# prashanthr05/bipedal-locomotion-framework

Hardware: AMD Instinct MI355X
Metric: DCM-MPC QP solves/sec (batch, horizon=100) at 1/2/4/8 MI355X (higher is better)
Workload: dtype f64; 1 GPU; configs[1]: batch=4096 DCM-MPC QPs per GPU, horizon=100, M=8 facet slots, fp64, one wavefront per QP; batch_per_gpu=4096, global_batch=4096, horizon=100, max_facets=8, parallelism=shard1 (independent problems)

## Files before the change

### bipedal-locomotion-framework_amd/csrc/dcm_mpc_as.hip

```cpp
#include "dcm_qp_common.h"
#include "dcm_mpc_ipm_body.h"

#include <stdlib.h>

#include <type_traits>

namespace blf {
namespace {
using namespace qp;

#ifdef BLF_STAMPS
__device__ unsigned long long g_as_stamps[32];
__device__ unsigned long long g_as_timeline[65536 * 4];
__device__ unsigned long long g_as32_timeline[65536 * 4];
#define AS_STAMP(t) unsigned long long t = __builtin_amdgcn_s_memtime()
#define AS_STAMP_ADD(slot, t0) \
    do { if (blockIdx.x < 64 && threadIdx.x == 0) atomicAdd(&g_as_stamps[slot], __builtin_amdgcn_s_memtime() - (t0)); } while (0)
#define AS_COUNT(slot) \
    do { if (blockIdx.x < 64 && threadIdx.x == 0) atomicAdd(&g_as_stamps[slot], 1ull); } while (0)
#else
#define AS_STAMP(t)
#define AS_STAMP_ADD(slot, t0)
#define AS_COUNT(slot)
#endif
// ... 64 lines not shown

constexpr int kAsMinWaves = 2;

template <class T>
struct Row {
    T x, y, b;
};

template <class T, class RS>
__device__ __forceinline__ Row<T> row(const RS& R, int i, int col)
{
    const int o = R.at(i, col);
    const auto a = R.A2[o];
    return {T(a.x), T(a.y), T(R.Bv[o])};
}

template <class T, class RS>
__device__ __forceinline__ Row<T> normal(const RS& R, int i, int col)
{
    const auto a = R.A2[R.at(i, col)];
    return {T(a.x), T(a.y), T(0)};
}

struct NoRows {};
template <int KPL>
struct RegRows {
    Row<float> v[KPL][kMaxFacets];
};
template <class RR>
constexpr bool kHasRows = !std::is_same<RR, NoRows>::value;

template <int KPL, class RS>
__device__ __forceinline__ void load_rows(RegRows<KPL>& rr, const RS& R, int N, int M, int lane)
{
#pragma unroll
    for (int j = 0; j < KPL; ++j) {
        const int col = KPL * lane + j < N ? R.col(j, lane) : 0;
#pragma unroll
        for (int i = 0; i < kMaxFacets; ++i) rr.v[j][i] = row<float>(R, i < M ? i : 0, col);
    }
}
template <int KPL, class RS>
__device__ __forceinline__ void load_rows(NoRows&, const RS&, int, int, int)
{
}



enum : int { kTreeKS = 0, kTreePad = 1, kTreeDpp = 2 };

template <int KPL, int TR>
__device__ __forceinline__ void assume_pad(int N)
{
    if (KPL == 2 && TR != kTreeDpp) __builtin_assume((TR == kTreePad) == (N <= 2 * kWave - 2));
}

template <class T, int KPL>
constexpr bool kPairFloat = sizeof(T) == 4 && KPL == 2;

template <int L, bool FWD, class T>
__device__ __forceinline__ void aff_level(T& g0, T& g1, T& g2, T& g3, T& e0, T& e1, int lane)
{
    T p0, p1, p2, p3, q0, q1;
    if constexpr (FWD) {
        p0 = tree_fwd<L>(g0); p1 = tree_fwd<L>(g1); p2 = tree_fwd<L>(g2);
        p3 = tree_fwd<L>(g3); q0 = tree_fwd<L>(e0); q1 = tree_fwd<L>(e1);
// ... 155 lines not shown
    K.qx0 = q0 * (K.x0 - K.xr0);
    K.qx1 = q1 * (K.x1 - K.xr1);
}

template <bool SEL, class T>
__device__ __forceinline__ void rc_knot(RcT<T>& e, bool own, T al, const T (&E)[3], const PT<T>& P)
{
    if constexpr (SEL) {
        const T a = own ? al : T(1);
        e.a0 = a; e.a1 = T(0); e.a2 = T(0); e.a3 = a;
        e.g0 = E[0]; e.g1 = E[1]; e.g2 = E[2];
        e.h0 = own ? P.Qw0 : T(0); e.h1 = T(0); e.h2 = own ? P.Qw1 : T(0);
    } else if (own) {
        e.a0 = al; e.a1 = T(0); e.a2 = T(0); e.a3 = al;
        e.g0 = E[0]; e.g1 = E[1]; e.g2 = E[2];
        e.h0 = P.Qw0; e.h1 = T(0); e.h2 = P.Qw1;
    } else {
        e.a0 = T(1); e.a1 = T(0); e.a2 = T(0); e.a3 = T(1);
        e.g0 = e.g1 = e.g2 = T(0);
        e.h0 = e.h1 = e.h2 = T(0);
    }
}

template <int KPL, int TR, class T>
__device__ __forceinline__ bool as_riccati(AKnotT<T> (&K)[KPL], const PT<T>& P, const T (&E)[KPL][3], int N,
                                           int lane)
{
    bool ok = true;
    RcT<T> e;
    rc_knot<kPairFloat<T, KPL>>(e, KPL * lane < N, K[0].al, E[0], P);
    if constexpr (KPL == 2) {
        RcT<T> e1;
        rc_knot<kPairFloat<T, KPL>>(e1, KPL * lane + 1 < N, K[1].al, E[1], P);
        ok = rc_combine(e, e1) && ok;
    }
    const int ln = opaque(lane);
    constexpr bool pad = KPL == 2 && TR == kTreePad;
    auto level = [&](int ad, RcT<T>& q) {
        q.a0 = bperm(ad, e.a0); q.a1 = bperm(ad, e.a1); q.a2 = bperm(ad, e.a2); q.a3 = bperm(ad, e.a3);
        q.g0 = bperm(ad, e.g0); q.g1 = bperm(ad, e.g1); q.g2 = bperm(ad, e.g2);
        q.h0 = bperm(ad, e.h0); q.h1 = bperm(ad, e.h1); q.h2 = bperm(ad, e.h2);
    };
    auto level1 = [&](RcT<T>& q) {
        constexpr int C = pad ? kNextKeep : kNextWrap;
        q.a0 = dpp1<C>(e.a0); q.a1 = dpp1<C>(e.a1); q.a2 = dpp1<C>(e.a2); q.a3 = dpp1<C>(e.a3);
        q.g0 = dpp1<C>(e.g0); q.g1 = dpp1<C>(e.g1); q.g2 = dpp1<C>(e.g2);
        q.h0 = dpp1<C>(e.h0); q.h1 = dpp1<C>(e.h1); q.h2 = dpp1<C>(e.h2);
    };
    if constexpr (TR == kTreeDpp) {
        rc_tree<0>(e, ok, lane);
        rc_tree<1>(e, ok, lane);
        rc_tree<2>(e, ok, lane);
        rc_tree<3>(e, ok, lane);
        rc_tree<4>(e, ok, lane);
        rc_tree<5>(e, ok, lane);
    } else {
        {
// ... 4 lines not shown
#pragma unroll
        for (int d = 2; d < kWave; d <<= 1) {
            RcT<T> q;
            level(ks_addr<pad, false>(ln, d), q);
            if (ks_has<pad, false>(ln, d)) ok = rc_combine(e, q) && ok;
        }
    }
    T P00, P01, P11;
    ok = rc_apply(e, P.Pw0, T(0), P.Pw1, P00, P01, P11) && ok;
    T Pn00 = dpp1<kNextWrap>(P00), Pn01 = dpp1<kNextWrap>(P01), Pn11 = dpp1<kNextWrap>(P11);
    if (lane == kWave - 1) {
        Pn00 = P.Pw0;
        Pn01 = T(0);
        Pn11 = P.Pw1;
    }
    constexpr int L = KPL - 1;
    K[L].P00 = Pn00;
    K[L].P01 = Pn01;
    K[L].P11 = Pn11;
    if constexpr (KPL == 2) {
        RcT<T> e1;
        rc_knot<kPairFloat<T, KPL>>(e1, KPL * lane + 1 < N, K[1].al, E[1], P);
        T o00, o01, o11;
        ok = rc_apply(e1, Pn00, Pn01, Pn11, o00, o01, o11) && ok;
        K[0].P00 = o00;
        K[0].P01 = o01;
        K[0].P11 = o11;
    }
#pragma unroll
    for (int j = 0; j < KPL; ++j) {
        if (KPL * lane + j == N - 1) {
            K[j].P00 = P.Pw0;
            K[j].P01 = T(0);
            K[j].P11 = P.Pw1;
        }
    }
    return ok;
}

template <int KPL, int TR, class T>
__device__ __forceinline__ void as_solve(const AKnotT<T> (&K)[KPL], const T (&g)[KPL][2], int N, int lane,
                                         T (&dr)[KPL][2], T (&dx)[KPL][2], T (&vn)[KPL][2])
{
    constexpr bool kSel = kPairFloat<T, KPL>;
    T G[KPL][4], c[KPL][2], y[KPL][2];
#pragma unroll
    for (int j = 0; j < KPL; ++j) {
        const bool own = KPL * lane + j < N;
        if constexpr (!kSel) {
            G[j][0] = G[j][1] = G[j][2] = G[j][3] = T(0);
            c[j][0] = c[j][1] = y[j][0] = y[j][1] = T(0);
        }
        if (kSel || own) {
            const AKnotT<T>& Kj = K[j];
            const T b2 = Kj.be * Kj.be;
            const T ab = Kj.al * Kj.be;
            const T m00 = FD2(Kj.P00, Kj.h00, Kj.P01, Kj.h01);
            const T m01 = FD2(Kj.P00, Kj.h01, Kj.P01, Kj.h11);
            const T m10 = FD2(Kj.P01, Kj.h00, Kj.P11, Kj.h01);
            const T m11 = FD2(Kj.P01, Kj.h01, Kj.P11, Kj.h11);
// ... 538 lines not shown

template <class T, class RS>
__device__ __forceinline__ void as_pass_h(AKnotT<T>& K, const PT<T>& P, const RS& R, int col, int pk,
                                          bool& okp, const Row<T>& na)
{
    const int pc = pk & 3, pi1 = (pk >> 2) & 15;
    const T b2 = K.be * K.be;
    const T B00 = fma(b2, K.P00, P.Rw0);
    const T B01 = b2 * K.P01;
    const T B11 = fma(b2, K.P11, P.Rw1);
    Row<T> a = na;
    if constexpr (!kCarryNormals<T>) a = normal<T>(R, pi1, opaque(col));
    const T u = a.y * a.y, v = a.x * a.x, q = a.x * a.y;
    const T detB = fma(B00, B11, -(B01 * B01));
    const T tbt = FD3(B00, u, B11, v, T(-2) * (B01 * q));
    const T den = pc == 0 ? detB : pc == 1 ? tbt : T(1);
    if (pc < 2 && (!(den > T(0)) || __builtin_isinf(den))) okp = false;
    const T id = T(1) / den;
    K.h00 = pc == 0 ? B11 * id : pc == 1 ? u * id : T(0);
    K.h01 = pc == 0 ? -(B01 * id) : pc == 1 ? -(q * id) : T(0);
    K.h11 = pc == 0 ? B00 * id : pc == 1 ? v * id : T(0);
}

template <class T, class RS, class RR>
__device__ __forceinline__ void as_certify(AKnotT<T>& K, const PT<T>& P, const RS& R, int col, int pk,
                                           T dx0, T dx1, T vn0, T vn1, T& l1o, T& l2o, bool& okp, bool& neg,
                                           bool& viol, bool bland, int& ndrop, int& nadd, const Row<T>& na,
                                           const Row<T>& ne, const RR& rr, int j)
{
    const int cx = opaque(col);
    const int pc = pk & 3, pi1 = (pk >> 2) & 15, pi2 = (pk >> 6) & 15;
    const T s0 = K.qx0 + vn0;
    const T s1 = K.qx1 + vn1;
    const T nu0 = FD3(K.P00, dx0, K.P01, dx1, s0);
    const T nu1 = FD3(K.P01, dx0, K.P11, dx1, s1);
    const T rh0 = P.Rw0 * (K.r0 - K.rr0);
    const T rh1 = P.Rw1 * (K.r1 - K.rr1);
    K.rh0 = nu0;
    K.rh1 = nu1;
    const T g0 = fma(K.be, nu0, -rh0);
    const T g1 = fma(K.be, nu1, -rh1);
    Row<T> a = na, e = ne;
    if constexpr (!kCarryNormals<T>) {
        a = normal<T>(R, pi1, cx);
        e = normal<T>(R, pi2, cx);
    }
    const T n = pc == 1 ? FD2(a.x, g0, a.y, g1) : T(1);
    const T d = pc == 1 ? FD2(a.x, a.x, a.y, a.y) : fma(a.x, e.y, -(a.y * e.x));
    const T qd = n / d;
    const T l1 = pc == 1 ? qd : pc == 2 ? fma(g0, e.y, -(e.x * g1)) * qd : T(0);
    const T l2 = pc == 2 ? fma(a.x, g1, -(g0 * a.y)) * qd : T(0);
    l1o = l1;
    l2o = l2;
    T tol_d = P.tol_d;
    if constexpr (sizeof(T) == 8) tol_d = P.tol_d * fmax(1.0, kTolDualRel * fmax(fabs(K.be * nu0), fabs(K.be * nu1)));
    bool bad = false;
    if (pc == 0) bad = !(fabs(g0) <= tol_d) || !(fabs(g1) <= tol_d);
    if (pc == 1) bad = !(fabs(fma(-l1, a.x, g0)) <= tol_d) || !(fabs(fma(-l1, a.y, g1)) <= tol_d);
    const bool n1 = pc >= 1 && !(l1 >= -tol_d);
    const bool n2 = pc == 2 && !(l2 >= -tol_d);
    const int dm = (n1 ? 1 << pi1 : 0) | (n2 ? 1 << pi2 : 0);
    if (bad || dm) okp = false;
    if (dm) neg = true;
    int dr = K.drop | dm, ad = K.add & ~dm;
    const int km = opaque(K.m);
    int vm = 0;
#pragma unroll
    for (int i0 = 0; i0 < RS::kMF; i0 += 4) {
        if (i0 >= km) break;
        Row<T> rv[4];
#pragma unroll
        for (int q = 0; q < 4; ++q) {
            if constexpr (kHasRows<RR>) {
                rv[q] = rr.v[j][i0 + q];
            } else {
                const int i = i0 + q < km ? i0 + q : 0;
                rv[q] = row<T>(R, i, cx);
            }
        }
#pragma unroll
        for (int q = 0; q < 4; ++q)
            if (!(FD2(rv[q].x, K.r0, rv[q].y, K.r1) - rv[q].b <= P.tol_p)) vm |= 1 << (i0 + q);
    }
    vm &= (1 << km) - 1;
    if (vm) {
        okp = false;
        viol = true;
        ad |= vm;
        dr &= ~vm;
    }
    ndrop = dr;
    nadd = ad;
    if (!bland) {
        K.drop = dr;
        K.add = ad;
    }
}

template <class T, class RS>
__device__ __forceinline__ void as_project(AKnotT<T>& K, const RS& R, int col, int pk)
{
    const int pc = pk & 3, pi1 = (pk >> 2) & 15;
    const Row<T> a = row<T>(R, pi1, opaque(col));
    const T aa = FD2(a.x, a.x, a.y, a.y);
    const T t = (FD2(a.x, K.r0, a.y, K.r1) - a.b) / aa;
// ... 32 lines not shown
                       K[j].xr1, K[j].w, wn[j], K[j].rh0, K[j].rh1, nn0[j], nn1[j], last, P.dt,
                       last ? P.Pw0 : P.Qw0, last ? P.Pw1 : P.Qw1, P.Rw0, P.Rw1, pk[j] & 3, a.x, a.y, K[j].d0,
                       K[j].d1, K[j].qx0, K[j].qx1, g[j][0], g[j][1]);
        }
    }
    as_solve<KPL, TR, double>(K, g, N, lane, dr, dx, vn);
#pragma unroll
    for (int j = 0; j < KPL; ++j) {
        if (KPL * lane + j < N) {
            K[j].rh0 = K[j].rh0 + FD3(K[j].P00, dx[j][0], K[j].P01, dx[j][1], K[j].qx0 + vn[j][0]);
            K[j].rh1 = K[j].rh1 + FD3(K[j].P01, dx[j][0], K[j].P11, dx[j][1], K[j].qx1 + vn[j][1]);
            K[j].r0 = K[j].r0 + dr[j][0];
            K[j].r1 = K[j].r1 + dr[j][1];
            K[j].x0 = K[j].x0 + dx[j][0];
            K[j].x1 = K[j].x1 + dx[j][1];
            as_project<double>(K[j], R, R.col(j, lane), pk[j]);
        }
    }
    }
}

template <int KPL, class T, class RS, class RR>
__device__ __forceinline__ void as_guess(AKnotT<T> (&K)[KPL], const RS& R, int NH, int N, int lane,
                                         const double* const (&lw)[KPL], double ws_floor, T thr, const RR& rr)
{
#pragma unroll
    for (int j = 0; j < KPL; ++j) {
        const int k = KPL * lane + j;
        if (k < N) {
            int gm = 0;
            if constexpr (kHasRows<RR>) {
#pragma unroll
                for (int i = 0; i < kMaxFacets; ++i) {
                    const Row<T> a = rr.v[j][i];
                    const T gr = FD2(a.x, K[j].r0, a.y, K[j].r1);
                    const T sl = a.b - gr;
                    if (i < K[j].m && sl < thr) gm |= 1 << i;
                }
            } else {
                const int col = R.col(j, lane);
                for (int i = 0; i < K[j].m; ++i) {
                    const Row<T> a = row<T>(R, i, col);
                    const T gr = FD2(a.x, K[j].r0, a.y, K[j].r1);
                    const T sl = a.b - gr;
                    if (sl < thr) gm |= 1 << i;
                    if (lw[j] && lw[j][i] > ws_floor) gm |= 1 << i;
                }
            }
            K[j].gm = gm;
        }
    }
}

template <class T>
__device__ __forceinline__ int as_cand(const AKnotT<T>& K)
{
    return ((K.gm & ~K.drop) | K.add) & ((1 << K.m) - 1);
}

template <int KPL, class T>
__device__ __forceinline__ decltype(auto) pass_params(const PT<T>& P)
{
    if constexpr (kPairFloat<T, KPL>) {
        PT<T> V = P;
        carry_in_vgpr(V.Rw0);
        carry_in_vgpr(V.Rw1);
        carry_in_vgpr(V.Qw0);
        carry_in_vgpr(V.Qw1);
        carry_in_vgpr(V.Pw0);
        carry_in_vgpr(V.Pw1);
        return V;
    } else {
        return (P);
    }
}

template <int KPL, int TR, class T, class RS, class RR>
__device__ __forceinline__ bool as_passes(AKnotT<T> (&K)[KPL], const PT<T>& Pin, const RS& R, int NH, int N,
                                          int lane, T xi00, T xi01, int (&pk)[KPL],
                                          T (&pl)[KPL][2], int count_slot, int sb, int handover, int& npass,
                                          const RR& rr)
{
    decltype(auto) P = pass_params<KPL>(Pin);
    T xk[KPL][2];
    as_xi_prev<KPL, T>(K, lane, xi00, xi01, xk);
    bool certified = false;
    constexpr bool kAnti = sizeof(T) == 8;
    constexpr int kMaxPass = kAnti ? kAsPasses : kGuessPasses;
    int pass = 0;
    for (; pass < kMaxPass; ++pass) {
        const bool bland = kAnti && pass >= kGuessPasses;
        AS_COUNT(count_slot);
        AS_STAMP(t_s);
        T sv[KPL][4];
        T E[KPL][3];
        int c0[KPL];
        bool okp = true;
        Row<T> na[KPL], ne[KPL];
#pragma unroll
        for (int j = 0; j < KPL; ++j) {
            const int k = KPL * lane + j;
            c0[j] = as_cand(K[j]);
            sv[j][0] = K[j].r0; sv[j][1] = K[j].r1; sv[j][2] = K[j].x0; sv[j][3] = K[j].x1;
            E[j][0] = E[j][1] = E[j][2] = T(0);
            pk[j] = 0;
            if (k < N)
                as_pass_setup<T>(K[j], P, R, R.col(j, lane), sv[j][0], sv[j][1], pk[j], E[j], okp, na[j], ne[j]);
        }
        AS_STAMP_ADD(sb + 0, t_s);
        AS_STAMP(t_r);
        okp = as_riccati<KPL, TR, T>(K, P, E, N, lane) && okp;
        AS_STAMP_ADD(sb + 1, t_r);
        AS_STAMP(t_h);
#pragma unroll
        for (int j = 0; j < KPL; ++j) {
            const int k = KPL * lane + j;
            if (k < N) {
                as_pass_h<T>(K[j], P, R, R.col(j, lane), opaque(pk[j]), okp, na[j]);
                as_residuals(K[j], P, k == N - 1, xk[j][0], xk[j][1]);
            }
        }
        AS_STAMP_ADD(sb + 2, t_h);
        bool neg = false, viol = false;
        int ndr[KPL], nad[KPL];
        {
            T g[KPL][2], dr[KPL][2], dx[KPL][2], vn[KPL][2];
#pragma unroll
            for (int j = 0; j < KPL; ++j) {
                g[j][0] = K[j].rh0;
                g[j][1] = K[j].rh1;
            }
            AS_STAMP(t_v);
            as_solve<KPL, TR, T>(K, g, N, lane, dr, dx, vn);
            AS_STAMP_ADD(sb + 3, t_v);
            AS_STAMP(t_c);
#pragma unroll
            for (int j = 0; j < KPL; ++j) {
                pl[j][0] = pl[j][1] = T(0);
                ndr[j] = K[j].drop;
                nad[j] = K[j].add;
                if (KPL * lane + j < N) {
                    K[j].r0 = K[j].r0 + dr[j][0];
                    K[j].r1 = K[j].r1 + dr[j][1];
                    K[j].x0 = K[j].x0 + dx[j][0];
                    K[j].x1 = K[j].x1 + dx[j][1];
                    if constexpr (sizeof(T) == 8) as_project<T>(K[j], R, R.col(j, lane), opaque(pk[j]));
                    as_certify<T>(K[j], P, R, R.col(j, lane), opaque(pk[j]), dx[j][0], dx[j][1], vn[j][0], vn[j][1],
                                  pl[j][0], pl[j][1], okp, neg, viol, kAnti && bland, ndr[j], nad[j], na[j], ne[j], rr, j);
                }
            }
            AS_STAMP_ADD(sb + 4, t_c);
        }
        AS_STAMP(t_o);
        if (__ballot(!okp) == 0) {
            certified = true;
            AS_STAMP_ADD(sb + 5, t_o);
            break;
        }
        if constexpr (kAnti) {
            if (bland) {
                bool ch[KPL];
#pragma unroll
                for (int j = 0; j < KPL; ++j) ch[j] = ndr[j] != K[j].drop || nad[j] != K[j].add;
                bool any = false;
#pragma unroll
                for (int j = 0; j < KPL; ++j) any = any || ch[j];
                const unsigned long long bl = __ballot(any);
                const int ls = bl ? __builtin_ctzll(bl) : -1;
                bool first = true;
#pragma unroll
                for (int j = 0; j < KPL; ++j) {
// ... 358 lines not shown
        Fj.m = 0;
        Fj.gm = Fj.drop = Fj.add = 0;
        Fj.w = Fj.be = 0.0f;
        Fj.rr0 = Fj.rr1 = Fj.xr0 = Fj.xr1 = 0.0f;
        Fj.rh0 = Fj.rh1 = Fj.d0 = Fj.d1 = Fj.qx0 = Fj.qx1 = 0.0f;
        Fj.P00 = Fj.P01 = Fj.P11 = Fj.h00 = Fj.h01 = Fj.h11 = 0.0f;
        kin[j] = KnotIn{0, 0.0, 0.0, 0.0, 0.0, 0.0};
        if (k < N) {
            const KnotIn in = knot_in<PH>(p, k, N, omega, xi_ref, vrp_ref, nfacets, ps, sPh);
            kin[j] = in;
            Fj.m = in.m < 0 ? 0 : in.m > M ? M : in.m;
            Fj.w = float(in.w);
            Fj.be = Pf.dt * Fj.w;
            Fj.rr0 = float(in.rr0);
            Fj.rr1 = float(in.rr1);
            Fj.xr0 = float(in.xr0);
            Fj.xr1 = float(in.xr1);
        }
        Fj.al = 1.0f + Fj.be;
        Fj.r0 = Fj.rr0; Fj.r1 = Fj.rr1;
        Fj.x0 = Fj.xr0; Fj.x1 = Fj.xr1;
    }
    const float xf00 = float(xi00), xf01 = float(xi01);
    if (kOverlap) stage_rows_issue<KPL, U>(Ain, bin, p, M, lane, 0, nA, va, vb);
    AS_STAMP_ADD(1, t_start);
    {
        AS_STAMP(t_q);
        as_lq_step<KPL, TR, float>(F, Pf, N, lane, xf00, xf01);
        if (kOverlap) stage_rows_commit<KPL, U, double, MF>(va, vb, M, S, NH, lane, 0, nA, A2d, Bv);
        __syncthreads();
        AS_STAMP_ADD(2, t_q);
        AS_STAMP(t_g);
        const double* const lw0[KPL] = {};
        std::conditional_t<MF == kMaxFacets && !PH, RegRows<KPL>, NoRows> rr;
        load_rows<KPL>(rr, R, N, M, lane);
        as_guess<KPL, float>(F, R, NH, N, lane, lw0, 0.0, 0.0f, rr);
        AS_STAMP_ADD(3, t_g);
        AS_STAMP(t_a);
        int pkf[KPL];
        float plf[KPL][2];
        cert32 = as_passes<KPL, TR, float>(F, Pf, R, NH, N, lane, xf00, xf01, pkf, plf, 12, 16, N / kHandoverDiv,
                                           npass32, rr);
        AS_STAMP_ADD(13, t_a);
    }
#pragma unroll
    for (int j = 0; j < KPL; ++j) cand[j] = as_cand(F[j]);

    AS_STAMP(t_b);
    const PT<double> Pd = params_d(P);
    AKnot K[KPL];
    bool bad = false;
#pragma unroll
    for (int j = 0; j < KPL; ++j) {
        const int k = KPL * lane + j;
        AKnot& Kj = K[j];
        knot_zero(Kj);
        if (k < N) {
            const KnotIn in = kin[j];
            Kj.m = in.m;
            Kj.w = in.w;
            Kj.rr0 = in.rr0;
            Kj.rr1 = in.rr1;
            Kj.xr0 = in.xr0;
            Kj.xr1 = in.xr1;
            if (Kj.m < 0 || Kj.m > M) {
// ... 11 lines not shown
    int status = 0;
    int npass = npass32;
    bool certified = false;
    double pl[KPL][2];
    int pk[KPL];
#pragma unroll
    for (int j = 0; j < KPL; ++j) {
        pl[j][0] = pl[j][1] = 0.0;
        pk[j] = 0;
    }
    if (__ballot(bad) != 0) {
        status = BLF_QP_BAD_FACETS;
        npass = 0;
#pragma unroll
        for (int j = 0; j < KPL; ++j) {
            K[j].r0 = K[j].rr0;
            K[j].r1 = K[j].rr1;
            K[j].x0 = K[j].xr0;
            K[j].x1 = K[j].xr1;
        }
    } else {
        const double* const lw0[KPL] = {};
        if (cert32) {
            as_guess<KPL, double>(K, R, NH, N, lane, lw0, 0.0, kGuessSlack, NoRows{});
        } else {
#pragma unroll
            for (int j = 0; j < KPL; ++j) K[j].gm = KPL * lane + j < N ? cand[j] : 0;
        }
        int npass64 = 0;
        certified = as_passes<KPL, TR, double>(K, Pd, R, NH, N, lane, xi00, xi01, pk, pl, 10, 4, -1, npass64, NoRows{});
        npass += npass64;
        if (!certified) {
#pragma unroll
            for (int j = 0; j < KPL; ++j) {
                if (KPL * lane + j < N) {
                    K[j].r0 = K[j].rr0;
                    K[j].r1 = K[j].rr1;
                    K[j].x0 = K[j].xr0;
                    K[j].x1 = K[j].xr1;
                }
            }
            if (!as_lq_step<KPL, TR, double>(K, Pd, N, lane, xi00, xi01)) status = BLF_QP_NUMERICAL;
        }
    }
    AS_STAMP_ADD(14, t_b);
    as_write_outputs<KPL, LAMOUT>(K, pk, pl, certified, status, p, N, M, lane, xi00, xi01, xi_out, vrp_out,
                                  status_out, iters_out, polished_out, lam_out, P.list, P.list_slot, P.list_cap,
                                  P.passes_out, npass, pend);
    if (PH && !certified && status == 0) ph_write_window<KPL>(ps, sPh, omega, A2d, Bv, p, N, M, S, NH, lane);
    AS_STAMP_ADD(0, t_start);
#ifdef BLF_STAMPS
    if (threadIdx.x == 0 && blockIdx.x < 65536) {
        g_as32_timeline[4 * blockIdx.x + 0] = t_rt0;
// ... 97 lines not shown
            Kj.rr0 = in.rr0;
            Kj.rr1 = in.rr1;
            Kj.xr0 = in.xr0;
            Kj.xr1 = in.xr1;
        }
    }
    if constexpr (!kWide) {
        if (PH) stage_rows_ph_issue<U>(ps, sPh, p, N, M, lane, va, vb);
        else stage_rows_issue<KPL, U>(Ain, bin, p, M, lane, 0, nA, va, vb);
    }
#pragma unroll
    for (int j = 0; j < KPL; ++j) {
        AKnot& Kj = K[j];
        if (KPL * lane + j < N) {
            if (Kj.m < 0 || Kj.m > M) {
                bad = true;
                Kj.m = 0;
            }
            Kj.be = Pd.dt * Kj.w;
        }
        Kj.al = 1.0 + Kj.be;
    }
    const bool any_bad = __ballot(bad) != 0;
    AS_STAMP_ADD(1, t_start);
    const LdsRows<double, MF> R{A2, Bv, S, NH};

    int status = 0;
    int npass = 0;
    bool certified = false;
    double pl[KPL][2];
    int pk[KPL];
#pragma unroll
    for (int j = 0; j < KPL; ++j) {
        pl[j][0] = pl[j][1] = 0.0;
        pk[j] = 0;
    }
    AS_STAMP(t_lq);
    {
        double g[KPL][4], f[KPL][2], xk[KPL][2], x[KPL][2];
#pragma unroll
        for (int j = 0; j < KPL; ++j) {
            const int k = KPL * lane + j;
            f[j][0] = f[j][1] = 0.0;
            if (k < N) {
                if (k == 0) {
                    f[j][0] = fma(K[j].al, xi00, -(K[j].be * K[j].r0));
// ... 6 lines not shown
            const double ga = k < N ? K[j].al : 0.0;
            g[j][0] = ga; g[j][1] = 0.0; g[j][2] = 0.0; g[j][3] = ga;
        }
        as_scan_forward<KPL, TR, double>(g, f, lane, x, xk);
#pragma unroll
        for (int j = 0; j < KPL; ++j) {
            K[j].x0 = x[j][0];
            K[j].x1 = x[j][1];
        }
    }
    if constexpr (!kWide) stage_rows_commit<KPL, U, double, MF>(va, vb, M, S, NH, lane, 0, nA, reinterpret_cast<double*>(A2), Bv);
    __syncthreads();
    AS_STAMP_ADD(2, t_lq);
    if (any_bad) {
        status = BLF_QP_BAD_FACETS;
    } else {
        AS_STAMP(t_g);
        const double* lw[KPL];
#pragma unroll
        for (int j = 0; j < KPL; ++j) {
            const int k = KPL * lane + j;
            lw[j] = (k < N && k + P.ws_shift < N) ? ws_lam + (p * N + k + P.ws_shift) * M : nullptr;
        }
        as_guess<KPL, double>(K, R, NH, N, lane, lw, P.ws_floor, 0.0, NoRows{});
        AS_STAMP_ADD(3, t_g);
        AS_STAMP(t_b);
        certified = as_passes<KPL, TR, double>(K, Pd, R, NH, N, lane, xi00, xi01, pk, pl, 10, 4, -1, npass, NoRows{});
        AS_STAMP_ADD(14, t_b);
    }
    if (!certified && status == 0) {
        pend = kPendingCold;
        __syncthreads();
        goto cold;
    }
    AS_STAMP(t_out);

    as_write_outputs<KPL, LAMOUT>(K, pk, pl, certified, status, p, N, M, lane, xi00, xi01, xi_out, vrp_out,
                                  status_out, iters_out, polished_out, lam_out, P.list, P.list_slot, P.list_cap,
                                  P.passes_out, npass);
    if (PH && !certified && status == 0)
        ph_write_window<KPL>(ps, sPh, omega, reinterpret_cast<const double*>(A2), Bv, p, N, M, S, NH, lane);
    AS_STAMP_ADD(11, t_out);
    AS_STAMP_ADD(15, t_start);
#ifdef BLF_STAMPS
    if (threadIdx.x == 0 && blockIdx.x < 65536) {
        g_as_timeline[4 * blockIdx.x + 0] = t_rt0;
        g_as_timeline[4 * blockIdx.x + 1] = __builtin_amdgcn_s_memrealtime();
        g_as_timeline[4 * blockIdx.x + 2] = t_start;
        g_as_timeline[4 * blockIdx.x + 3] = __builtin_amdgcn_s_memtime();
    }
// ... 133 lines not shown
```

### bipedal-locomotion-framework_amd/csrc/dcm_qp_common.h

```cpp
#pragma once
#include "blf_internal.h"

namespace blf {
namespace qp {

constexpr int kGuessPasses = 8;
constexpr int kAsPasses = 12;


constexpr int kPending = -1;
constexpr int kPendingCold = -2;

struct KParams {
    int N, M, max_iter;
    int ws_shift;
    const int32_t* ws_status;
    double dt, Qw0, Qw1, Rw0, Rw1, Pw0, Pw1, tol_mu, tol_p, tol_d;
    double tol_polish;
    double ws_floor;
    int stage2;
    int32_t* list;
    int list_slot;
    int list_cap;
    int32_t* passes_out;
// ... 204 lines not shown
}

template <int L, class T>
__device__ __forceinline__ T tree_bwd(T x)
{
    return tree_src<L, false>(x);
}

template <int L, bool FWD>
__device__ __forceinline__ bool tree_has(int lane)
{
    const int r = lane >> 4;
    if constexpr (FWD) {
        if constexpr (L < 4) return (lane & 15) >= (1 << L);
        else if constexpr (L == 4) return (r & 1) != 0;
        else return r >= 2;
    } else {
        if constexpr (L < 4) return (lane & 15) + (1 << L) <= 15;
        else if constexpr (L == 4) return (r & 1) == 0;
        else return r < 2;
    }
}

#define FD2(a, b, c, d) fma((a), (b), (c) * (d))
#define FD3(a, b, c, d, e) fma((a), (b), fma((c), (d), (e)))

static __device__ __forceinline__ int vertex_pair(const double2* A2, const double* Bo, int bs, int N,
                                                            int kx, int km, int cm, double tol_p, int& pi1,
                                                            int& pi2)
{
    for (int x = 0; x < km; ++x) {
        if (!((cm >> x) & 1)) continue;
        for (int y = x + 1; y < km; ++y) {
            if (!((cm >> y) & 1)) continue;
            const double2 a = A2[x * N + kx];
            const double2 e = A2[y * N + kx];
            const double ba = Bo[(x * N + kx) * bs], be = Bo[(y * N + kx) * bs];
            const double det = fma(a.x, e.y, -(a.y * e.x));
            const double aa = FD2(a.x, a.x, a.y, a.y), ee = FD2(e.x, e.x, e.y, e.y);
            if (!(det * det > 1e-18 * (aa * ee))) continue;
            const double idet = 1.0 / det;
            const double v0 = fma(ba, e.y, -(a.y * be)) * idet;
            const double v1 = fma(a.x, be, -(ba * e.x)) * idet;
            bool feas = true;
            for (int l = 0; l < km; ++l) {
                const double2 f = A2[l * N + kx];
                if (!(FD2(f.x, v0, f.y, v1) - Bo[(l * N + kx) * bs] <= tol_p)) feas = false;
            }
            if (feas) {
                pi1 = x;
                pi2 = y;
                return 2;
            }
        }
    }
    return 3;
}

#define COMPOSE(a0, a1, a2, a3, b0, b1, b2, b3, c0, c1, e0, e1)                 \
    do {                                                                         \
        const double n0_ = FD2(a0, b0, a1, b2);                                  \
        const double n1_ = FD2(a0, b1, a1, b3);                                  \
        const double n2_ = FD2(a2, b0, a3, b2);                                  \
        const double n3_ = FD2(a2, b1, a3, b3);                                  \
        const double m0_ = FD3(a0, c0, a1, c1, e0);                              \
        const double m1_ = FD3(a2, c0, a3, c1, e1);                              \
        a0 = n0_; a1 = n1_; a2 = n2_; a3 = n3_; e0 = m0_; e1 = m1_;               \
    } while (0)

template <class T>
struct RcT {
    T a0, a1, a2, a3, g0, g1, g2, h0, h1, h2;
};
using Rc = RcT<double>;

template <class T>
__device__ __forceinline__ bool rc_combine(RcT<T>& e, const RcT<T>& q)
{
    const T one = T(1);
    const T T00 = FD3(e.g0, q.h0, e.g1, q.h1, one);
    const T T01 = FD2(e.g0, q.h1, e.g1, q.h2);
    const T T10 = FD2(e.g1, q.h0, e.g2, q.h1);
    const T T11 = FD3(e.g1, q.h1, e.g2, q.h2, one);
    const T detT = fma(T00, T11, -(T01 * T10));
    const bool ok = (detT > T(0)) && !__builtin_isinf(detT);
    const T it = one / detT;
    const T Up00 = FD2(T11, e.a0, -T01, e.a2);
    const T Up01 = FD2(T11, e.a1, -T01, e.a3);
    const T Up10 = FD2(-T10, e.a0, T00, e.a2);
    const T Up11 = FD2(-T10, e.a1, T00, e.a3);
    const T Vp00 = FD2(q.a0, T11, q.a1, -T10);
    const T Vp01 = FD2(q.a0, -T01, q.a1, T00);
    const T Vp10 = FD2(q.a2, T11, q.a3, -T10);
    const T Vp11 = FD2(q.a2, -T01, q.a3, T00);
    const T Xp00 = FD2(Vp00, e.g0, Vp01, e.g1);
    const T Xp01 = FD2(Vp00, e.g1, Vp01, e.g2);
    const T Xp10 = FD2(Vp10, e.g0, Vp11, e.g1);
    const T Xp11 = FD2(Vp10, e.g1, Vp11, e.g2);
    const T Y00 = FD2(q.h0, e.a0, q.h1, e.a2);
    const T Y01 = FD2(q.h0, e.a1, q.h1, e.a3);
    const T Y10 = FD2(q.h1, e.a0, q.h2, e.a2);
    const T Y11 = FD2(q.h1, e.a1, q.h2, e.a3);
    const T gp0 = FD2(Xp00, q.a0, Xp01, q.a1);
    const T gp1 = FD2(Xp00, q.a2, Xp01, q.a3);
    const T gp2 = FD2(Xp10, q.a2, Xp11, q.a3);
    const T U00 = Up00 * it, U01 = Up01 * it, U10 = Up10 * it, U11 = Up11 * it;
    RcT<T> r;
    r.a0 = FD2(q.a0, U00, q.a1, U10);
    r.a1 = FD2(q.a0, U01, q.a1, U11);
    r.a2 = FD2(q.a2, U00, q.a3, U10);
    r.a3 = FD2(q.a2, U01, q.a3, U11);
    r.h0 = FD3(U00, Y00, U10, Y10, e.h0);
    r.h1 = FD3(U00, Y01, U10, Y11, e.h1);
    r.h2 = FD3(U01, Y01, U11, Y11, e.h2);
    r.g0 = fma(gp0, it, q.g0);
    r.g1 = fma(gp1, it, q.g1);
    r.g2 = fma(gp2, it, q.g2);
    e = r;
    return ok;
}

template <class T>
__device__ __forceinline__ bool rc_apply(const RcT<T>& e, T P00, T P01, T P11, T& o00, T& o01, T& o11)
{
    const T one = T(1);
    const T S00 = FD3(e.g0, P00, e.g1, P01, one);
    const T S01 = FD2(e.g0, P01, e.g1, P11);
    const T S10 = FD2(e.g1, P00, e.g2, P01);
    const T S11 = FD3(e.g1, P01, e.g2, P11, one);
    const T detS = fma(S00, S11, -(S01 * S10));
    const bool ok = (detS > T(0)) && !__builtin_isinf(detS);
    const T is = one / detS;
    const T Wp00 = FD2(P00, S11, P01, -S10);
    const T Wp01 = FD2(P00, -S01, P01, S00);
    const T Wp10 = FD2(P01, S11, P11, -S10);
    const T Wp11 = FD2(P01, -S01, P11, S00);
    const T Zp00 = FD2(Wp00, e.a0, Wp01, e.a2);
    const T Zp01 = FD2(Wp00, e.a1, Wp01, e.a3);
    const T Zp10 = FD2(Wp10, e.a0, Wp11, e.a2);
    const T Zp11 = FD2(Wp10, e.a1, Wp11, e.a3);
    o00 = fma(FD2(e.a0, Zp00, e.a2, Zp10), is, e.h0);
    o01 = fma(FD2(e.a0, Zp01, e.a2, Zp11), is, e.h1);
    o11 = fma(FD2(e.a1, Zp01, e.a3, Zp11), is, e.h2);
    return ok;
}

template <class T>
struct RcD {
    T a0, a3, g0, g2, h0, h2;
};

template <bool ISO, class T>
__device__ __forceinline__ bool rcd_combine(RcD<T>& e, const RcD<T>& q)
{
    const T one = T(1);
    const T T00 = fma(e.g0, q.h0, one);
    const T T11 = ISO ? T00 : fma(e.g2, q.h2, one);
    const T detT = T00 * T11;
    const bool ok = (detT > T(0)) && !__builtin_isinf(detT);
    const T it = one / detT;
    RcD<T> r;
    {
        const T Up00 = T11 * e.a0;
        const T Vp00 = q.a0 * T11;
        const T Xp00 = Vp00 * e.g0;
        const T Y00 = q.h0 * e.a0;
        const T gp0 = Xp00 * q.a0;
        const T U00 = Up00 * it;
// ... 99 lines not shown
```

Before: 45.52 million QP/s.

## Add leaf-specialised Riccati combine and wave-wide facet slot bound to skip unused rows

Adds specialised leaf forms of the Riccati combine and apply that exploit the diagonal structure of single-knot elements (a1=a2=0, h1=0). It first runs the sweep with them, checks the result with a wave ballot and a finiteness checksum, and falls back to the general sweep when that check fails. Separately, it computes a wave-wide maximum active facet count via ballots. Row loading, guess and certification loops use it to skip facet slots beyond that bound. The aim is to cut ALU work and row loads, at the cost of a possible second sweep on fallback and extra ballot overhead. The Riccati helpers also move into a new header usable from host code.

After: 45.44 million QP/s, median of 2. About the same (-0.2%).

```diff
diff --git a/bipedal-locomotion-framework_amd/csrc/dcm_mpc_as.hip b/bipedal-locomotion-framework_amd/csrc/dcm_mpc_as.hip
--- a/bipedal-locomotion-framework_amd/csrc/dcm_mpc_as.hip
+++ b/bipedal-locomotion-framework_amd/csrc/dcm_mpc_as.hip
@@ -110,6 +110,23 @@
     return {T(a.x), T(a.y), T(0)};
 }
 
+template <class T, int KPL, int MF, bool PH>
+constexpr bool kLeafPass = KPL == 2 && MF == kMaxFacets && (sizeof(T) == 4 || !PH);
+template <int KPL, int MF>
+constexpr bool kSlotBound = KPL == 2 && MF == kMaxFacets;
+
+template <int KPL, class KN>
+__device__ __forceinline__ int slot_bound(const KN (&K)[KPL])
+{
+    int mm = K[0].m;
+    if constexpr (KPL == 2) mm = max(mm, K[1].m);
+    int mmax = 0;
+#pragma unroll
+    for (int b = 16; b >= 1; b >>= 1)
+        if (__ballot(mm >= (mmax | b)) != 0) mmax |= b;
+    return mmax;
+}
+
 struct NoRows {};
 template <int KPL>
 struct RegRows {
@@ -119,17 +136,21 @@
 constexpr bool kHasRows = !std::is_same<RR, NoRows>::value;
 
 template <int KPL, class RS>
-__device__ __forceinline__ void load_rows(RegRows<KPL>& rr, const RS& R, int N, int M, int lane)
-{
+__device__ __forceinline__ void load_rows(RegRows<KPL>& rr, const RS& R, int N, int M, int lane, int mmax)
+{
+    constexpr bool kSB = kSlotBound<KPL, RS::kMF>;
 #pragma unroll
     for (int j = 0; j < KPL; ++j) {
         const int col = KPL * lane + j < N ? R.col(j, lane) : 0;
 #pragma unroll
-        for (int i = 0; i < kMaxFacets; ++i) rr.v[j][i] = row<float>(R, i < M ? i : 0, col);
+        for (int i = 0; i < kMaxFacets; ++i) {
+            if (kSB && i >= 4 && (i & ~1) >= mmax) break;
+            rr.v[j][i] = row<float>(R, i < M ? i : 0, col);
+        }
     }
 }
 template <int KPL, class RS>
-__device__ __forceinline__ void load_rows(NoRows&, const RS&, int, int, int)
+__device__ __forceinline__ void load_rows(NoRows&, const RS&, int, int, int, int)
 {
 }
 
@@ -331,17 +352,20 @@
     }
 }
 
-template <int KPL, int TR, class T>
-__device__ __forceinline__ bool as_riccati(AKnotT<T> (&K)[KPL], const PT<T>& P, const T (&E)[KPL][3], int N,
-                                           int lane)
-{
+template <int KPL, int TR, bool LEAF, class T>
+__device__ __forceinline__ bool as_riccati_sweep(AKnotT<T> (&K)[KPL], const PT<T>& P, const T (&E)[KPL][3], int N,
+                                                 int lane, T& chk)
+{
+    static_assert(!LEAF || KPL == 2, "the leaf forms are the knot pair's");
     bool ok = true;
     RcT<T> e;
+    T sp_c = T(0), sp_a = T(0);
     rc_knot<kPairFloat<T, KPL>>(e, KPL * lane < N, K[0].al, E[0], P);
     if constexpr (KPL == 2) {
         RcT<T> e1;
         rc_knot<kPairFloat<T, KPL>>(e1, KPL * lane + 1 < N, K[1].al, E[1], P);
-        ok = rc_combine(e, e1) && ok;
+        if constexpr (LEAF) ok = rc_combine_leaves(e, e1, sp_c) && ok;
+        else ok = rc_combine(e, e1) && ok;
     }
     const int ln = opaque(lane);
     constexpr bool pad = KPL == 2 && TR == kTreePad;
@@ -392,7 +416,12 @@
         RcT<T> e1;
         rc_knot<kPairFloat<T, KPL>>(e1, KPL * lane + 1 < N, K[1].al, E[1], P);
         T o00, o01, o11;
-        ok = rc_apply(e1, Pn00, Pn01, Pn11, o00, o01, o11) && ok;
+        if constexpr (LEAF) {
+            ok = rc_apply_leaf(e1, Pn00, Pn01, Pn11, o00, o01, o11, sp_a) && ok;
+            chk = (((P00 + P01) + P11) + ((o00 + o01) + o11)) + (sp_c + sp_a);
+        } else {
+            ok = rc_apply(e1, Pn00, Pn01, Pn11, o00, o01, o11) && ok;
+        }
         K[0].P00 = o00;
         K[0].P01 = o01;
         K[0].P11 = o11;
@@ -406,6 +435,21 @@
         }
     }
     return ok;
+}
+
+__device__ __forceinline__ bool nonfinite(float v) { return __builtin_amdgcn_classf(v, 0x207); }
+__device__ __forceinline__ bool nonfinite(double v) { return __builtin_amdgcn_class(v, 0x207); }
+
+template <int KPL, int TR, class T, bool LEAF = false>
+__device__ __forceinline__ bool as_riccati(AKnotT<T> (&K)[KPL], const PT<T>& P, const T (&E)[KPL][3], int N,
+                                           int lane)
+{
+    T chk = T(0);
+    if constexpr (LEAF) {
+        const bool ok = as_riccati_sweep<KPL, TR, true, T>(K, P, E, N, lane, chk);
+        if (__ballot(!ok || nonfinite(chk)) == 0) return true;
+    }
+    return as_riccati_sweep<KPL, TR, false, T>(K, P, E, N, lane, chk);
 }
 
 template <int KPL, int TR, class T>
@@ -990,11 +1034,11 @@
     K.h11 = pc == 0 ? B00 * id : pc == 1 ? v * id : T(0);
 }
 
-template <class T, class RS, class RR>
+template <class T, bool SB, class RS, class RR>
 __device__ __forceinline__ void as_certify(AKnotT<T>& K, const PT<T>& P, const RS& R, int col, int pk,
                                            T dx0, T dx1, T vn0, T vn1, T& l1o, T& l2o, bool& okp, bool& neg,
                                            bool& viol, bool bland, int& ndrop, int& nadd, const Row<T>& na,
-                                           const Row<T>& ne, const RR& rr, int j)
+                                           const Row<T>& ne, const RR& rr, int j, int mmax)
 {
     const int cx = opaque(col);
     const int pc = pk & 3, pi1 = (pk >> 2) & 15, pi2 = (pk >> 6) & 15;
@@ -1033,22 +1077,43 @@
     int dr = K.drop | dm, ad = K.add & ~dm;
     const int km = opaque(K.m);
     int vm = 0;
-#pragma unroll
-    for (int i0 = 0; i0 < RS::kMF; i0 += 4) {
-        if (i0 >= km) break;
-        Row<T> rv[4];
-#pragma unroll
-        for (int q = 0; q < 4; ++q) {
-            if constexpr (kHasRows<RR>) {
-                rv[q] = rr.v[j][i0 + q];
-            } else {
-                const int i = i0 + q < km ? i0 + q : 0;
-                rv[q] = row<T>(R, i, cx);
+    if constexpr (SB) {
+        auto group = [&](int i0, auto n) {
+            Row<T> rv[n()];
+#pragma unroll
+            for (int q = 0; q < n(); ++q) {
+                if constexpr (kHasRows<RR>) {
+                    rv[q] = rr.v[j][i0 + q];
+                } else {
+                    const int i = i0 + q < km ? i0 + q : 0;
+                    rv[q] = row<T>(R, i, cx);
+                }
             }
-        }
-#pragma unroll
-        for (int q = 0; q < 4; ++q)
-            if (!(FD2(rv[q].x, K.r0, rv[q].y, K.r1) - rv[q].b <= P.tol_p)) vm |= 1 << (i0 + q);
+#pragma unroll
+            for (int q = 0; q < n(); ++q)
+                if (!(FD2(rv[q].x, K.r0, rv[q].y, K.r1) - rv[q].b <= P.tol_p)) vm |= 1 << (i0 + q);
+        };
+        if (mmax > 0) group(0, std::integral_constant<int, 4>{});
+        if (mmax > 4) group(4, std::integral_constant<int, 2>{});
+        if (mmax > 6) group(6, std::integral_constant<int, 2>{});
+    } else {
+#pragma unroll
+        for (int i0 = 0; i0 < RS::kMF; i0 += 4) {
+            if (i0 >= km) break;
+            Row<T> rv[4];
+#pragma unroll
+            for (int q = 0; q < 4; ++q) {
+                if constexpr (kHasRows<RR>) {
+                    rv[q] = rr.v[j][i0 + q];
+                } else {
+                    const int i = i0 + q < km ? i0 + q : 0;
+                    rv[q] = row<T>(R, i, cx);
+                }
+            }
+#pragma unroll
+            for (int q = 0; q < 4; ++q)
+                if (!(FD2(rv[q].x, K.r0, rv[q].y, K.r1) - rv[q].b <= P.tol_p)) vm |= 1 << (i0 + q);
+        }
     }
     vm &= (1 << km) - 1;
     if (vm) {
@@ -1127,8 +1192,10 @@
 
 template <int KPL, class T, class RS, class RR>
 __device__ __forceinline__ void as_guess(AKnotT<T> (&K)[KPL], const RS& R, int NH, int N, int lane,
-                                         const double* const (&lw)[KPL], double ws_floor, T thr, const RR& rr)
-{
+                                         const double* const (&lw)[KPL], double ws_floor, T thr, const RR& rr,
+                                         int mmax)
+{
+    constexpr bool kSB = kSlotBound<KPL, RS::kMF>;
 #pragma unroll
     for (int j = 0; j < KPL; ++j) {
         const int k = KPL * lane + j;
@@ -1137,10 +1204,21 @@
             if constexpr (kHasRows<RR>) {
 #pragma unroll
                 for (int i = 0; i < kMaxFacets; ++i) {
+                    if (kSB && i >= 4 && (i & ~1) >= mmax) break;
                     const Row<T> a = rr.v[j][i];
                     const T gr = FD2(a.x, K[j].r0, a.y, K[j].r1);
                     const T sl = a.b - gr;
                     if (i < K[j].m && sl < thr) gm |= 1 << i;
+                }
+            } else if constexpr (kSB) {
+                const int col = R.col(j, lane);
+                for (int i = 0; i < mmax; ++i) {
+                    const bool has = i < K[j].m;
+                    const Row<T> a = row<T>(R, has ? i : 0, col);
+                    const T gr = FD2(a.x, K[j].r0, a.y, K[j].r1);
+                    const T sl = a.b - gr;
+                    if (has && sl < thr) gm |= 1 << i;
+                    if (has && lw[j] && lw[j][i] > ws_floor) gm |= 1 << i;
                 }
             } else {
                 const int col = R.col(j, lane);
@@ -1180,11 +1258,11 @@
     }
 }
 
-template <int KPL, int TR, class T, class RS, class RR>
+template <int KPL, int TR, bool LEAF, class T, class RS, class RR>
 __device__ __forceinline__ bool as_passes(AKnotT<T> (&K)[KPL], const PT<T>& Pin, const RS& R, int NH, int N,
                                           int lane, T xi00, T xi01, int (&pk)[KPL],
                                           T (&pl)[KPL][2], int count_slot, int sb, int handover, int& npass,
-                                          const RR& rr)
+                                          const RR& rr, int mmax)
 {
     decltype(auto) P = pass_params<KPL>(Pin);
     T xk[KPL][2];
@@ -1214,7 +1292,7 @@
         }
         AS_STAMP_ADD(sb + 0, t_s);
         AS_STAMP(t_r);
-        okp = as_riccati<KPL, TR, T>(K, P, E, N, lane) && okp;
+        okp = as_riccati<KPL, TR, T, LEAF>(K, P, E, N, lane) && okp;
         AS_STAMP_ADD(sb + 1, t_r);
         AS_STAMP(t_h);
 #pragma unroll
@@ -1250,8 +1328,9 @@
                     K[j].x0 = K[j].x0 + dx[j][0];
                     K[j].x1 = K[j].x1 + dx[j][1];
                     if constexpr (sizeof(T) == 8) as_project<T>(K[j], R, R.col(j, lane), opaque(pk[j]));
-                    as_certify<T>(K[j], P, R, R.col(j, lane), opaque(pk[j]), dx[j][0], dx[j][1], vn[j][0], vn[j][1],
-                                  pl[j][0], pl[j][1], okp, neg, viol, kAnti && bland, ndr[j], nad[j], na[j], ne[j], rr, j);
+                    as_certify<T, kSlotBound<KPL, RS::kMF>>(K[j], P, R, R.col(j, lane), opaque(pk[j]), dx[j][0], dx[j][1],
+                                                            vn[j][0], vn[j][1], pl[j][0], pl[j][1], okp, neg, viol,
+                                                            kAnti && bland, ndr[j], nad[j], na[j], ne[j], rr, j, mmax);
                 }
             }
             AS_STAMP_ADD(sb + 4, t_c);
@@ -1656,6 +1735,8 @@
         Fj.x0 = Fj.xr0; Fj.x1 = Fj.xr1;
     }
     const float xf00 = float(xi00), xf01 = float(xi01);
+    int mmax = MF;
+    if constexpr (kSlotBound<KPL, MF>) mmax = slot_bound(F);
     if (kOverlap) stage_rows_issue<KPL, U>(Ain, bin, p, M, lane, 0, nA, va, vb);
     AS_STAMP_ADD(1, t_start);
     {
@@ -1667,14 +1748,14 @@
         AS_STAMP(t_g);
         const double* const lw0[KPL] = {};
         std::conditional_t<MF == kMaxFacets && !PH, RegRows<KPL>, NoRows> rr;
-        load_rows<KPL>(rr, R, N, M, lane);
-        as_guess<KPL, float>(F, R, NH, N, lane, lw0, 0.0, 0.0f, rr);
+        load_rows<KPL>(rr, R, N, M, lane, mmax);
+        as_guess<KPL, float>(F, R, NH, N, lane, lw0, 0.0, 0.0f, rr, mmax);
         AS_STAMP_ADD(3, t_g);
         AS_STAMP(t_a);
         int pkf[KPL];
         float plf[KPL][2];
-        cert32 = as_passes<KPL, TR, float>(F, Pf, R, NH, N, lane, xf00, xf01, pkf, plf, 12, 16, N / kHandoverDiv,
-                                           npass32, rr);
+        cert32 = as_passes<KPL, TR, kLeafPass<float, KPL, MF, PH>, float>(F, Pf, R, NH, N, lane, xf00, xf01, pkf, plf, 12, 16, N / kHandoverDiv,
+                                           npass32, rr, mmax);
         AS_STAMP_ADD(13, t_a);
     }
 #pragma unroll
@@ -1732,13 +1813,13 @@
     } else {
         const double* const lw0[KPL] = {};
         if (cert32) {
-            as_guess<KPL, double>(K, R, NH, N, lane, lw0, 0.0, kGuessSlack, NoRows{});
+            as_guess<KPL, double>(K, R, NH, N, lane, lw0, 0.0, kGuessSlack, NoRows{}, mmax);
         } else {
 #pragma unroll
             for (int j = 0; j < KPL; ++j) K[j].gm = KPL * lane + j < N ? cand[j] : 0;
         }
         int npass64 = 0;
-        certified = as_passes<KPL, TR, double>(K, Pd, R, NH, N, lane, xi00, xi01, pk, pl, 10, 4, -1, npass64, NoRows{});
+        certified = as_passes<KPL, TR, kLeafPass<double, KPL, MF, PH>, double>(K, Pd, R, NH, N, lane, xi00, xi01, pk, pl, 10, 4, -1, npass64, NoRows{}, mmax);
         npass += npass64;
         if (!certified) {
 #pragma unroll
@@ -1882,6 +1963,8 @@
         Kj.al = 1.0 + Kj.be;
     }
     const bool any_bad = __ballot(bad) != 0;
+    int mmax = MF;
+    if constexpr (kSlotBound<KPL, MF>) mmax = slot_bound(K);
     AS_STAMP_ADD(1, t_start);
     const LdsRows<double, MF> R{A2, Bv, S, NH};
 
@@ -1934,10 +2017,10 @@
             const int k = KPL * lane + j;
             lw[j] = (k < N && k + P.ws_shift < N) ? ws_lam + (p * N + k + P.ws_shift) * M : nullptr;
         }
-        as_guess<KPL, double>(K, R, NH, N, lane, lw, P.ws_floor, 0.0, NoRows{});
+        as_guess<KPL, double>(K, R, NH, N, lane, lw, P.ws_floor, 0.0, NoRows{}, mmax);
         AS_STAMP_ADD(3, t_g);
         AS_STAMP(t_b);
-        certified = as_passes<KPL, TR, double>(K, Pd, R, NH, N, lane, xi00, xi01, pk, pl, 10, 4, -1, npass, NoRows{});
+        certified = as_passes<KPL, TR, kLeafPass<double, KPL, MF, PH>, double>(K, Pd, R, NH, N, lane, xi00, xi01, pk, pl, 10, 4, -1, npass, NoRows{}, mmax);
         AS_STAMP_ADD(14, t_b);
     }
     if (!certified && status == 0) {
diff --git a/bipedal-locomotion-framework_amd/csrc/dcm_qp_common.h b/bipedal-locomotion-framework_amd/csrc/dcm_qp_common.h
--- a/bipedal-locomotion-framework_amd/csrc/dcm_qp_common.h
+++ b/bipedal-locomotion-framework_amd/csrc/dcm_qp_common.h
@@ -1,5 +1,6 @@
 #pragma once
 #include "blf_internal.h"
+#include "dcm_rc.h"
 
 namespace blf {
 namespace qp {
@@ -250,8 +251,6 @@
     }
 }
 
-#define FD2(a, b, c, d) fma((a), (b), (c) * (d))
-#define FD3(a, b, c, d, e) fma((a), (b), fma((c), (d), (e)))
 
 static __device__ __forceinline__ int vertex_pair(const double2* A2, const double* Bo, int bs, int N,
                                                             int kx, int km, int cm, double tol_p, int& pi1,
@@ -296,82 +295,6 @@
         a0 = n0_; a1 = n1_; a2 = n2_; a3 = n3_; e0 = m0_; e1 = m1_;               \
     } while (0)
 
-template <class T>
-struct RcT {
-    T a0, a1, a2, a3, g0, g1, g2, h0, h1, h2;
-};
-using Rc = RcT<double>;
-
-template <class T>
-__device__ __forceinline__ bool rc_combine(RcT<T>& e, const RcT<T>& q)
-{
-    const T one = T(1);
-    const T T00 = FD3(e.g0, q.h0, e.g1, q.h1, one);
-    const T T01 = FD2(e.g0, q.h1, e.g1, q.h2);
-    const T T10 = FD2(e.g1, q.h0, e.g2, q.h1);
-    const T T11 = FD3(e.g1, q.h1, e.g2, q.h2, one);
-    const T detT = fma(T00, T11, -(T01 * T10));
-    const bool ok = (detT > T(0)) && !__builtin_isinf(detT);
-    const T it = one / detT;
-    const T Up00 = FD2(T11, e.a0, -T01, e.a2);
-    const T Up01 = FD2(T11, e.a1, -T01, e.a3);
-    const T Up10 = FD2(-T10, e.a0, T00, e.a2);
-    const T Up11 = FD2(-T10, e.a1, T00, e.a3);
-    const T Vp00 = FD2(q.a0, T11, q.a1, -T10);
-    const T Vp01 = FD2(q.a0, -T01, q.a1, T00);
-    const T Vp10 = FD2(q.a2, T11, q.a3, -T10);
-    const T Vp11 = FD2(q.a2, -T01, q.a3, T00);
-    const T Xp00 = FD2(Vp00, e.g0, Vp01, e.g1);
-    const T Xp01 = FD2(Vp00, e.g1, Vp01, e.g2);
-    const T Xp10 = FD2(Vp10, e.g0, Vp11, e.g1);
-    const T Xp11 = FD2(Vp10, e.g1, Vp11, e.g2);
-    const T Y00 = FD2(q.h0, e.a0, q.h1, e.a2);
-    const T Y01 = FD2(q.h0, e.a1, q.h1, e.a3);
-    const T Y10 = FD2(q.h1, e.a0, q.h2, e.a2);
-    const T Y11 = FD2(q.h1, e.a1, q.h2, e.a3);
-    const T gp0 = FD2(Xp00, q.a0, Xp01, q.a1);
-    const T gp1 = FD2(Xp00, q.a2, Xp01, q.a3);
-    const T gp2 = FD2(Xp10, q.a2, Xp11, q.a3);
-    const T U00 = Up00 * it, U01 = Up01 * it, U10 = Up10 * it, U11 = Up11 * it;
-    RcT<T> r;
-    r.a0 = FD2(q.a0, U00, q.a1, U10);
-    r.a1 = FD2(q.a0, U01, q.a1, U11);
-    r.a2 = FD2(q.a2, U00, q.a3, U10);
-    r.a3 = FD2(q.a2, U01, q.a3, U11);
-    r.h0 = FD3(U00, Y00, U10, Y10, e.h0);
-    r.h1 = FD3(U00, Y01, U10, Y11, e.h1);
-    r.h2 = FD3(U01, Y01, U11, Y11, e.h2);
-    r.g0 = fma(gp0, it, q.g0);
-    r.g1 = fma(gp1, it, q.g1);
-    r.g2 = fma(gp2, it, q.g2);
-    e = r;
-    return ok;
-}
-
-template <class T>
-__device__ __forceinline__ bool rc_apply(const RcT<T>& e, T P00, T P01, T P11, T& o00, T& o01, T& o11)
-{
-    const T one = T(1);
-    const T S00 = FD3(e.g0, P00, e.g1, P01, one);
-    const T S01 = FD2(e.g0, P01, e.g1, P11);
-    const T S10 = FD2(e.g1, P00, e.g2, P01);
-    const T S11 = FD3(e.g1, P01, e.g2, P11, one);
-    const T detS = fma(S00, S11, -(S01 * S10));
-    const bool ok = (detS > T(0)) && !__builtin_isinf(detS);
-    const T is = one / detS;
-    const T Wp00 = FD2(P00, S11, P01, -S10);
-    const T Wp01 = FD2(P00, -S01, P01, S00);
-    const T Wp10 = FD2(P01, S11, P11, -S10);
-    const T Wp11 = FD2(P01, -S01, P11, S00);
-    const T Zp00 = FD2(Wp00, e.a0, Wp01, e.a2);
-    const T Zp01 = FD2(Wp00, e.a1, Wp01, e.a3);
-    const T Zp10 = FD2(Wp10, e.a0, Wp11, e.a2);
-    const T Zp11 = FD2(Wp10, e.a1, Wp11, e.a3);
-    o00 = fma(FD2(e.a0, Zp00, e.a2, Zp10), is, e.h0);
-    o01 = fma(FD2(e.a0, Zp01, e.a2, Zp11), is, e.h1);
-    o11 = fma(FD2(e.a1, Zp01, e.a3, Zp11), is, e.h2);
-    return ok;
-}
 
 template <class T>
 struct RcD {
diff --git a/bipedal-locomotion-framework_amd/csrc/dcm_rc.h b/bipedal-locomotion-framework_amd/csrc/dcm_rc.h
--- /dev/null
+++ b/bipedal-locomotion-framework_amd/csrc/dcm_rc.h
@@ -0,0 +1,171 @@
+#pragma once
+
+#if defined(__HIPCC__)
+#define BLF_RC_FN __device__ __forceinline__
+#else
+#include <cmath>
+#define BLF_RC_FN inline
+#endif
+
+#define FD2(a, b, c, d) fma((a), (b), (c) * (d))
+#define FD3(a, b, c, d, e) fma((a), (b), fma((c), (d), (e)))
+
+namespace blf {
+namespace qp {
+
+#if !defined(__HIPCC__)
+using std::fma;
+#endif
+
+template <class T>
+struct RcT {
+    T a0, a1, a2, a3, g0, g1, g2, h0, h1, h2;
+};
+using Rc = RcT<double>;
+
+template <class T>
+BLF_RC_FN bool rc_combine(RcT<T>& e, const RcT<T>& q)
+{
+    const T one = T(1);
+    const T T00 = FD3(e.g0, q.h0, e.g1, q.h1, one);
+    const T T01 = FD2(e.g0, q.h1, e.g1, q.h2);
+    const T T10 = FD2(e.g1, q.h0, e.g2, q.h1);
+    const T T11 = FD3(e.g1, q.h1, e.g2, q.h2, one);
+    const T detT = fma(T00, T11, -(T01 * T10));
+    const bool ok = (detT > T(0)) && !__builtin_isinf(detT);
+    const T it = one / detT;
+    const T Up00 = FD2(T11, e.a0, -T01, e.a2);
+    const T Up01 = FD2(T11, e.a1, -T01, e.a3);
+    const T Up10 = FD2(-T10, e.a0, T00, e.a2);
+    const T Up11 = FD2(-T10, e.a1, T00, e.a3);
+    const T Vp00 = FD2(q.a0, T11, q.a1, -T10);
+    const T Vp01 = FD2(q.a0, -T01, q.a1, T00);
+    const T Vp10 = FD2(q.a2, T11, q.a3, -T10);
+    const T Vp11 = FD2(q.a2, -T01, q.a3, T00);
+    const T Xp00 = FD2(Vp00, e.g0, Vp01, e.g1);
+    const T Xp01 = FD2(Vp00, e.g1, Vp01, e.g2);
+    const T Xp10 = FD2(Vp10, e.g0, Vp11, e.g1);
+    const T Xp11 = FD2(Vp10, e.g1, Vp11, e.g2);
+    const T Y00 = FD2(q.h0, e.a0, q.h1, e.a2);
+    const T Y01 = FD2(q.h0, e.a1, q.h1, e.a3);
+    const T Y10 = FD2(q.h1, e.a0, q.h2, e.a2);
+    const T Y11 = FD2(q.h1, e.a1, q.h2, e.a3);
+    const T gp0 = FD2(Xp00, q.a0, Xp01, q.a1);
+    const T gp1 = FD2(Xp00, q.a2, Xp01, q.a3);
+    const T gp2 = FD2(Xp10, q.a2, Xp11, q.a3);
+    const T U00 = Up00 * it, U01 = Up01 * it, U10 = Up10 * it, U11 = Up11 * it;
+    RcT<T> r;
+    r.a0 = FD2(q.a0, U00, q.a1, U10);
+    r.a1 = FD2(q.a0, U01, q.a1, U11);
+    r.a2 = FD2(q.a2, U00, q.a3, U10);
+    r.a3 = FD2(q.a2, U01, q.a3, U11);
+    r.h0 = FD3(U00, Y00, U10, Y10, e.h0);
+    r.h1 = FD3(U00, Y01, U10, Y11, e.h1);
+    r.h2 = FD3(U01, Y01, U11, Y11, e.h2);
+    r.g0 = fma(gp0, it, q.g0);
+    r.g1 = fma(gp1, it, q.g1);
+    r.g2 = fma(gp2, it, q.g2);
+    e = r;
+    return ok;
+}
+
+template <class T>
+BLF_RC_FN bool rc_apply(const RcT<T>& e, T P00, T P01, T P11, T& o00, T& o01, T& o11)
+{
+    const T one = T(1);
+    const T S00 = FD3(e.g0, P00, e.g1, P01, one);
+    const T S01 = FD2(e.g0, P01, e.g1, P11);
+    const T S10 = FD2(e.g1, P00, e.g2, P01);
+    const T S11 = FD3(e.g1, P01, e.g2, P11, one);
+    const T detS = fma(S00, S11, -(S01 * S10));
+    const bool ok = (detS > T(0)) && !__builtin_isinf(detS);
+    const T is = one / detS;
+    const T Wp00 = FD2(P00, S11, P01, -S10);
+    const T Wp01 = FD2(P00, -S01, P01, S00);
+    const T Wp10 = FD2(P01, S11, P11, -S10);
+    const T Wp11 = FD2(P01, -S01, P11, S00);
+    const T Zp00 = FD2(Wp00, e.a0, Wp01, e.a2);
+    const T Zp01 = FD2(Wp00, e.a1, Wp01, e.a3);
+    const T Zp10 = FD2(Wp10, e.a0, Wp11, e.a2);
+    const T Zp11 = FD2(Wp10, e.a1, Wp11, e.a3);
+    o00 = fma(FD2(e.a0, Zp00, e.a2, Zp10), is, e.h0);
+    o01 = fma(FD2(e.a0, Zp01, e.a2, Zp11), is, e.h1);
+    o11 = fma(FD2(e.a1, Zp01, e.a3, Zp11), is, e.h2);
+    return ok;
+}
+
+template <class T>
+BLF_RC_FN bool rc_combine_leaves(RcT<T>& e, const RcT<T>& q, T& spare)
+{
+    const T one = T(1);
+    const T ae = e.a0, aq = q.a0;
+    const T T00 = fma(e.g0, q.h0, one);
+    const T T01 = e.g1 * q.h2;
+    const T T10 = e.g1 * q.h0;
+    const T T11 = fma(e.g2, q.h2, one);
+    const T detT = fma(T00, T11, -(T01 * T10));
+    const bool ok = (detT > T(0)) && !__builtin_isinf(detT);
+    const T it = one / detT;
+    const T Up00 = T11 * ae;
+    const T Up01 = -T01 * ae;
+    const T Up10 = -T10 * ae;
+    const T Up11 = T00 * ae;
+    const T Vp00 = aq * T11;
+    const T Vp01 = aq * -T01;
+    const T Vp10 = aq * -T10;
+    const T Vp11 = aq * T00;
+    const T Xp00 = FD2(Vp00, e.g0, Vp01, e.g1);
+    const T Xp01 = FD2(Vp00, e.g1, Vp01, e.g2);
+    const T Xp10 = FD2(Vp10, e.g0, Vp11, e.g1);
+    const T Xp11 = FD2(Vp10, e.g1, Vp11, e.g2);
+    const T Y00 = q.h0 * ae;
+    const T Y11 = q.h2 * ae;
+    const T gp0 = Xp00 * aq;
+    const T gp1 = Xp01 * aq;
+    const T gp2 = Xp11 * aq;
+    const T U00 = Up00 * it, U01 = Up01 * it, U10 = Up10 * it, U11 = Up11 * it;
+    RcT<T> r;
+    r.a0 = aq * U00;
+    r.a1 = aq * U01;
+    r.a2 = aq * U10;
+    r.a3 = aq * U11;
+    r.h0 = fma(U00, Y00, e.h0);
+    r.h1 = fma(U10, Y11, e.h1);
+    r.h2 = fma(U11, Y11, e.h2);
+    r.g0 = fma(gp0, it, q.g0);
+    r.g1 = fma(gp1, it, q.g1);
+    r.g2 = fma(gp2, it, q.g2);
+    spare = Xp10;
+    e = r;
+    return ok;
+}
+
+template <class T>
+BLF_RC_FN bool rc_apply_leaf(const RcT<T>& e, T P00, T P01, T P11, T& o00, T& o01, T& o11, T& spare)
+{
+    const T one = T(1);
+    const T al = e.a0;
+    const T S00 = FD3(e.g0, P00, e.g1, P01, one);
+    const T S01 = FD2(e.g0, P01, e.g1, P11);
+    const T S10 = FD2(e.g1, P00, e.g2, P01);
+    const T S11 = FD3(e.g1, P01, e.g2, P11, one);
+    const T detS = fma(S00, S11, -(S01 * S10));
+    const bool ok = (detS > T(0)) && !__builtin_isinf(detS);
+    const T is = one / detS;
+    const T Wp00 = FD2(P00, S11, P01, -S10);
+    const T Wp01 = FD2(P00, -S01, P01, S00);
+    const T Wp10 = FD2(P01, S11, P11, -S10);
+    const T Wp11 = FD2(P01, -S01, P11, S00);
+    const T Zp00 = Wp00 * al;
+    const T Zp01 = Wp01 * al;
+    const T Zp10 = Wp10 * al;
+    const T Zp11 = Wp11 * al;
+    o00 = fma(al * Zp00, is, e.h0);
+    o01 = fma(al * Zp01, is, e.h1);
+    o11 = fma(al * Zp11, is, e.h2);
+    spare = Zp10;
+    return ok;
+}
+
+}
+}
```
